# omroot/DeepLearningInAssetPricing_PaperReplication

Measured on AMD Instinct MI355X. Metric: epochs/sec (3-phase GAN), higher is better.
Workload: dtype bf16; 1 GPU; model=Chen-Pelger-Zhu GAN: LSTM[4] + SDF FFN[64,64] + 8 tanh moments, global_batch=1, seq_len=240, panel=T=240/60/300 N=3000 F=46 M=178, bench_config=real, wide_layer0=False, models_per_gpu=1, parallelism=ensemble-dp1, backend=none

## Files before the change

### csrc/k_tbwd.hip

```cpp
#include <algorithm>
#include <type_traits>
#include "common.h"
#include "layout.h"
#include "mlp.h"
#include "tower_dev.h"

typedef short s16x4 __attribute__((ext_vector_type(4)));
typedef uint32_t u32x2 __attribute__((ext_vector_type(2)));
#define LDS3 __attribute__((address_space(3)))

__device__ long long g_tb_ts[8];

namespace {

constexpr int kImg = 4096;
constexpr int kImgs = 3;

DLAP_DEV int img_off(int r, int k) {
  const int f = ((r >> 1) & 1) | (((r >> 3) & 1) << 1), g = (r & 1) << 1;
  return r * 128 + ((((k >> 2) ^ f)) << 5) + (((k & 3) ^ g) << 3);
}

struct ImgMap {
  int wt[4];
  int wx[2];
  int rd[4];
};

DLAP_DEV bf16x8 img_get_sliced(const char* img, int u) {
  const int l = lane_id(), q = l >> 4, n = l & 15;
  const int off = img_off(4 * q + (n >> 2), 4 * u + (n & 3));
  const s16x4 lo = __builtin_amdgcn_ds_read_tr16_b64_v4i16((LDS3 s16x4*)(const_cast<char*>(img) + off));
  const s16x4 hi = __builtin_amdgcn_ds_read_tr16_b64_v4i16((LDS3 s16x4*)(const_cast<char*>(img) + off + 2048));
  typedef short s16x8 __attribute__((ext_vector_type(8)));
  const s16x8 v{lo[0], lo[1], lo[2], lo[3], hi[0], hi[1], hi[2], hi[3]};
  return __builtin_bit_cast(bf16x8, v);
}

DLAP_DEV ImgMap img_map() {
  ImgMap m;
  const int l = lane_id(), q = l >> 4, n = l & 15;
#pragma unroll
  for (int c = 0; c < 4; ++c) m.wt[c] = img_off(n, 4 * c + q);
#pragma unroll
  for (int s = 0; s < 2; ++s) m.wx[s] = img_off(n, 8 * s + 2 * q);
#pragma unroll
  for (int u = 0; u < 4; ++u) m.rd[u] = img_off(8 * q + (n >> 2), 4 * u + (n & 3));
  return m;
}

DLAP_DEV void img_put_t(char* img, const ImgMap& m, const bf16x8 (&f)[2][2]) {
#pragma unroll
  for (int b = 0; b < 2; ++b)
#pragma unroll
    for (int s = 0; s < 2; ++s) {
      const u32x4 v = __builtin_bit_cast(u32x4, f[b][s]);
      *(LDS3 u32x2*)(img + 2048 * b + m.wt[2 * s]) = u32x2{v[0], v[1]};
      *(LDS3 u32x2*)(img + 2048 * b + m.wt[2 * s + 1]) = u32x2{v[2], v[3]};
    }
}
DLAP_DEV void img_put_x(char* img, const ImgMap& m, const bf16x8 (&x)[2][2]) {
#pragma unroll
  for (int b = 0; b < 2; ++b)
#pragma unroll
    for (int s = 0; s < 2; ++s)
      *(LDS3 u32x4*)(img + 2048 * b + m.wx[s]) = __builtin_bit_cast(u32x4, x[b][s]);
}
DLAP_DEV bf16x8 img_get(const char* img, const ImgMap& m, int u) {
  const s16x4 lo = __builtin_amdgcn_ds_read_tr16_b64_v4i16((LDS3 s16x4*)(const_cast<char*>(img) + m.rd[u]));
  const s16x4 hi = __builtin_amdgcn_ds_read_tr16_b64_v4i16((LDS3 s16x4*)(const_cast<char*>(img) + m.rd[u] + 512));
  typedef short s16x8 __attribute__((ext_vector_type(8)));
  const s16x8 v{lo[0], lo[1], lo[2], lo[3], hi[0], hi[1], hi[2], hi[3]};
  return __builtin_bit_cast(bf16x8, v);
}

DLAP_DEV void mma_acc(f32x4& acc, const bf16x8& a, const bf16x8& b) {
  asm("v_mfma_f32_16x16x32_bf16 %0, %1, %2, %0" : "+a"(acc) : "v"(a), "v"(b));
}
DLAP_DEV void acc_fence4(f32x4& a0, f32x4& a1, f32x4& a2, f32x4& a3) {
  asm volatile("s_nop 7\n\ts_nop 7\n\ts_nop 7" : "+a"(a0), "+a"(a1), "+a"(a2), "+a"(a3));
}

__host__ __device__ inline size_t tb_img_base(const MlpDims& D) { return (lds_bytes_of(D) + 15) & ~(size_t)15; }
size_t tb_lds_bytes(const MlpDims& D) {
  const size_t loop = tb_img_base(D) + (size_t)4 * kImgs * kImg;
  const size_t red = (size_t)4 * 4096 * sizeof(float);
  return std::max(loop, red);
}

template <int NL, bool RES>
struct TbW;
template <int NL>
struct TbW<NL, true> {
  bf16x8 w0_[8];
  bf16x8 wf_[NL > 1 ? NL - 1 : 1][8];
  bf16x8 wb_[NL > 1 ? NL - 1 : 1][8];
  bf16x8 wpp_[2];
  DLAP_DEV TbW(const bf16x8* lds, const MlpDims& D) {
#pragma unroll
    for (int k = 0; k < 8; ++k) w0_[k] = ldsf(lds, D.s_fwd0 + k);
#pragma unroll
    for (int j = 0; j + 1 < NL; ++j)
#pragma unroll
      for (int k = 0; k < 8; ++k) {
        wf_[j][k] = ldsf(lds, D.s_fwd + 8 * j + k);
        wb_[j][k] = ldsf(lds, D.s_bwd + 8 * j + k);
      }
#pragma unroll
    for (int k = 0; k < 2; ++k) wpp_[k] = ldsf(lds, D.s_upp + k);
  }
  DLAP_DEV bf16x8 w0(int k) const { return w0_[k]; }
  DLAP_DEV bf16x8 wf(int j, int k) const { return wf_[j][k]; }
  DLAP_DEV bf16x8 wb(int j, int k) const { return wb_[j][k]; }
  DLAP_DEV bf16x8 wpp(int k) const { return wpp_[k]; }
};
template <int NL>
struct TbW<NL, false> {
  const bf16x8* lds;
  const MlpDims& D;
  DLAP_DEV TbW(const bf16x8* l, const MlpDims& d) : lds(l), D(d) {}
  DLAP_DEV bf16x8 w0(int k) const { return ldsf(lds, D.s_fwd0 + k); }
  DLAP_DEV bf16x8 wf(int j, int k) const { return ldsf(lds, D.s_fwd + 8 * j + k); }
  DLAP_DEV bf16x8 wb(int j, int k) const { return ldsf(lds, D.s_bwd + 8 * j + k); }
  DLAP_DEV bf16x8 wpp(int k) const { return ldsf(lds, D.s_upp + k); }
};
template <int NL>
constexpr bool kTbRes = NL <= 2;

template <typename WG>
DLAP_DEV void tb_chain(WG&& wget, const bf16x8 (&pf)[2][2], f32x4 (&acc)[2][4], const float* bias) {
  const int q = lane_id() >> 4;
#pragma unroll
  for (int u = 0; u < 4; ++u) {
    f32x4 c0 = bias ? ld4(bias + 16 * u + 4 * q) : zero4(), c1 = c0;
#pragma unroll
    for (int s = 0; s < 2; ++s) {
      const bf16x8 w = wget(2 * u + s);
      c0 = PrecBF16::mma(w, pf[0][s], c0);
      c1 = PrecBF16::mma(w, pf[1][s], c1);
    }
    acc[0][u] = c0; acc[1][u] = c1;
  }
}

DLAP_DEV void tb_finish(const MlpJob& J, const MlpDims& D, int tile, TileIn<PrecBF16, 2>& in, bf16x8 (&xf)[2][2],
                        const float* spp) {
  const int l = lane_id(), q = l >> 4;
  const int c0 = 32 + 8 * q - D.ppc;
  const bool ins = D.Dm > 0 && c0 >= 0;
  const int ca = max(c0, 0), cb = min(ca + 4, D.ppst - 4);
#pragma unroll
  for (int b = 0; b < 2; ++b) {
    const int r = tile * 32 + 16 * b + (l & 15);
    if (r >= J.R) in.dw[b] = 0.f;
    xf[b][0] = in.x[b][0];
    const float* row = spp + in.ti[b].x * D.ppst;
    const f32x4 v0 = ld4(row + ca), v1 = ld4(row + cb);
    const bf16x8 f = PrecBF16::pack(v0, c0 + 4 < D.ppst ? v1 : zero4());
    xf[b][1] = ins ? f : in.x[b][1];
  }
}

template <int NL>
struct TbState {
  f32x4 dW[NL][4][4];
  f32x4 gb[4];
  f32x4 gwo[4];
  float gbo;
};

template <int NL, bool ZIN, class TI>
DLAP_DEV void tb_tile(const MlpJob& J, const MlpDims& D, const TbW<NL, kTbRes<NL>>& W, const float* aux, const float* spp,
                      char* img, const ImgMap& im, int tile, TI& in, const uint32_t (&kw)[NL],
                      TbState<NL>& S) {
  using P = PrecBF16;
  using Frag = bf16x8;
  const int lane = lane_id(), q = lane >> 4;
  const float* auxt = aux;
  char* ximg = img;
  char* aimg = img + kImg;
  char* zimg = img + 2 * kImg;
  Frag xf[2][2];
  f32x4 a[2][4];
  if constexpr (ZIN) {
    const RowInfo ri = finish_ztile<1>(J, tile, in);
#pragma unroll
    for (int b = 0; b < 2; ++b) {
      xf[b][0] = pp_xfrag<P>(spp, D.ppst, ri.t[b], 0, D);
      xf[b][1] = P::zero();
    }
    img_put_x(ximg, im, xf);
    __builtin_amdgcn_sched_barrier(0);
    zin_sdf0(in.zs, ri, spp, D.ppst, auxt, D, a);
  } else {
    tb_finish(J, D, tile, in, xf, spp);
    img_put_x(ximg, im, xf);
    __builtin_amdgcn_sched_barrier(0);
#pragma unroll
    for (int u = 0; u < 4; ++u) {
      const f32x4 bias = ld4(auxt + D.a_sb + 16 * u + 4 * q);
      f32x4 c0 = bias, c1 = bias;
#pragma unroll
      for (int s = 0; s < 2; ++s) {
        const Frag w = W.w0(2 * u + s);
        c0 = P::mma(w, xf[0][s], c0);
        c1 = P::mma(w, xf[1][s], c1);
      }
      a[0][u] = c0; a[1][u] = c1;
    }
  }
  Frag act[NL][2][2];
  act_tile<P, 4, true>(a, kw[0], act[0]);
#pragma unroll
  for (int j = 1; j < NL; ++j) {
    tb_chain([&](int k) { return W.wf(j - 1, k); }, act[j - 1], a, auxt + D.a_sb + 64 * j);
    act_tile<P, 4, true>(a, kw[j], act[j]);
    __builtin_amdgcn_sched_barrier(0);
  }
  const float dw0 = in.dw[0], dw1 = in.dw[1];
  Frag dzf[2][2];
  {
    f32x4 t[2][4];
#pragma unroll
    for (int u = 0; u < 4; ++u) {
      const f32x4 ww = ld4(auxt + D.a_wo + 16 * u + 4 * q);
      t[0][u] = dw0 * ww;
      t[1][u] = dw1 * ww;
    }
    gate_tile<P, 4>(t, act[NL - 1], dzf);
  }
#pragma unroll
  for (int b = 0; b < 2; ++b)
#pragma unroll
    for (int s = 0; s < 2; ++s) {
      f32x4 lo, hi;
      P::unpack(act[NL - 1][b][s], lo, hi);
      const float d = b ? dw1 : dw0;
      S.gwo[2 * s] += d * lo;
      S.gwo[2 * s + 1] += d * hi;
    }
  S.gbo += q == 0 ? dw0 + dw1 : 0.f;
  __builtin_amdgcn_sched_barrier(0);
#pragma unroll
  for (int j = NL - 1; j >= 0; --j) {
    img_put_t(zimg, im, dzf);
    if (j > 0) img_put_t(aimg, im, act[j - 1]);
    Frag dzN[4];
#pragma unroll
    for (int u = 0; u < 4; ++u) dzN[u] = img_get(zimg, im, u);
    const Frag oh = make_onehot<P>(j);
#pragma unroll
    for (int u = 0; u < 4; ++u) {
      if constexpr (NL == 4) S.gb[u] = P::mma(dzN[u], oh, S.gb[u]);
      else mma_acc(S.gb[u], dzN[u], oh);
    }
#pragma unroll
    for (int v = 0; v < 4; ++v) {
      if (ZIN && j == 0 && v > 0) break;
      const Frag aN = img_get(j > 0 ? aimg : ximg, im, v);
#pragma unroll
      for (int u = 0; u < 4; ++u) mma_acc(S.dW[j][u][v], dzN[u], aN);
    }
    if constexpr (ZIN) {
      if (j == 0) {
        const auto dzo = gp(reinterpret_cast<bf16x8*>(J.dz_out)) + (size_t)tile * 4 * 64 + lane_id();
#pragma unroll
        for (int u = 0; u < 4; ++u) dzo[u * 64] = img_get_sliced(zimg, u);
      }
    }
    __builtin_amdgcn_sched_barrier(0);
    if (j > 0) {
      f32x4 da[2][4];
      tb_chain([&](int k) { return W.wb(j - 1, k); }, dzf, da, nullptr);
      gate_tile<P, 4>(da, act[j - 1], dzf);
    } else if (D.nrnn > 0) {
      f32x4 c[2];
#pragma unroll
      for (int b = 0; b < 2; ++b) {
        c[b] = zero4();
#pragma unroll
        for (int s = 0; s < 2; ++s) c[b] = P::mma(W.wpp(s), dzf[b][s], c[b]);
      }
#pragma unroll
      for (int b = 0; b < 2; ++b) {
        const int row = tile * 32 + 16 * b + (lane & 15);
#pragma unroll
        for (int r = 0; r < 4; ++r) {
          const int d = 4 * q + r;
          if (d < D.Dm && row < J.R) *gp32(J.u_out, (uint32_t)(row * D.Dm + d)) = c[b][r];
        }
      }
    }
  }
}

template <int NL>
DLAP_DEV void tb_issue_kw(const DLAP_GLOBAL uint32_t* gbase, int tile, int ntiles, uint32_t (&kw)[NL]) {
  const int lane = lane_id();
#pragma unroll
  for (int j = 0; j < NL; ++j)
    kw[j] = (gbase && tile < ntiles) ? *at32(gbase, (uint32_t)((tile * NL + j) * 64 + lane)) : 0xFFFFFFFFu;
}

template <int NL>
DLAP_DEV void tb_reduce_store(const MlpJob& J, char* smem, int slab_stride, TbState<NL>& S) {
  const int lane = lane_id(), wave = threadIdx.x >> 6, q = lane >> 4, n = lane & 15;
  float* red = reinterpret_cast<float*>(smem);
  const auto slab = gp(J.slab) + (size_t)(J.slab_base + blockIdx.x) * slab_stride;
#pragma unroll
  for (int j = 0; j < NL; ++j)
#pragma unroll
    for (int u = 0; u < 4; ++u) acc_fence4(S.dW[j][u][0], S.dW[j][u][1], S.dW[j][u][2], S.dW[j][u][3]);
  if constexpr (NL < 4) acc_fence4(S.gb[0], S.gb[1], S.gb[2], S.gb[3]);
  __syncthreads();
#pragma unroll
  for (int j = 0; j < NL; ++j) {
    if (j) __syncthreads();
    float* mine = red + wave * 4096;
#pragma unroll
    for (int u = 0; u < 4; ++u)
#pragma unroll
      for (int v = 0; v < 4; ++v) *reinterpret_cast<f32x4*>(mine + ((4 * u + v) * 64 + lane) * 4) = S.dW[j][u][v];
    __syncthreads();
#pragma unroll
    for (int k = 0; k < 4; ++k) {
      const int pos = (wave * 256 + k * 64 + lane) * 4;
      const f32x4 a = *reinterpret_cast<const f32x4*>(red + pos), b = *reinterpret_cast<const f32x4*>(red + 4096 + pos);
      const f32x4 c = *reinterpret_cast<const f32x4*>(red + 8192 + pos), d = *reinterpret_cast<const f32x4*>(red + 12288 + pos);
      *(DLAP_GLOBAL f32x4*)(slab + j * 4096 + pos) = (a + b) + (c + d);
    }
  }
  __syncthreads();
  float* ex = red + wave * SLAB_EXTRA;
  for (int x = lane; x < SLAB_EXTRA; x += 64) ex[x] = 0.f;
#pragma unroll
  for (int u = 0; u < 4; ++u)
#pragma unroll
    for (int r = 0; r < 4; ++r) {
      const int o = 16 * u + 4 * q + r;
      if (n < NL) ex[64 * n + o] = S.gb[u][r];
      float v = S.gwo[u][r];
      v += __shfl_xor(v, 1, 64); v += __shfl_xor(v, 2, 64);
      v += __shfl_xor(v, 4, 64); v += __shfl_xor(v, 8, 64);
      if (n == 0) ex[64 * DLAP_MAXL + o] = v;
    }
  const float bo = wave_sum(S.gbo);
  if (lane == 0) ex[64 * DLAP_MAXL + 64] = bo;
  __syncthreads();
  for (int x = threadIdx.x; x < SLAB_EXTRA; x += blockDim.x)
    slab[NL * 4096 + x] = (red[x] + red[SLAB_EXTRA + x]) + (red[2 * SLAB_EXTRA + x] + red[3 * SLAB_EXTRA + x]);
}

template <int NL, bool ZIN>
__global__ __launch_bounds__(256, 1) void k_tbwd_sdf(const MlpJob* __restrict__ jobs, MlpDims D, int slab_stride) {
  using P = PrecBF16;
  extern __shared__ __attribute__((aligned(16))) char smem[];
  const MlpJob J = jobs[blockIdx.y];
  bf16x8* lds = reinterpret_cast<bf16x8*>(smem);
  float* aux = aux_lds_ptr(smem, D);
  float* spp = pp_lds_ptr(smem, D);
  const int wave = threadIdx.x >> 6;
  char* img = smem + tb_img_base(D) + (size_t)wave * kImgs * kImg;
  const ImgMap im = img_map();
  const bool tsb = blockIdx.y == 0 && threadIdx.x == 0 && (blockIdx.x == 0 || blockIdx.x == gridDim.x - 1);
  const int tso = blockIdx.x == 0 ? 0 : 4;
  if (tsb) g_tb_ts[tso] = wall_clock64();
  const int ntiles = (J.R + 31) >> 5;
  const int stride = J.nslab * 4;
  const int t0 = blockIdx.x * 4 + wave;
  TbState<NL> S;
#pragma unroll
  for (int j = 0; j < NL; ++j)
#pragma unroll
    for (int u = 0; u < 4; ++u)
#pragma unroll
      for (int v = 0; v < 4; ++v) S.dW[j][u][v] = zero4();
#pragma unroll
  for (int u = 0; u < 4; ++u) { S.gb[u] = zero4(); S.gwo[u] = zero4(); }
  S.gbo = 0.f;
  uint32_t stp_raw = *gp(J.step ? reinterpret_cast<const uint32_t*>(J.step)
                                : reinterpret_cast<const uint32_t*>(J.rowti));
  using TI = std::conditional_t<ZIN, ZTile<1>, TileIn<P, 2>>;
  auto issue = [&](int t, TI& in) {
    if constexpr (ZIN) issue_ztile<1, true>(J, D, t, in, true, false);
    else issue_tile<P, 2, true>(J, t, in);
  };
  TI s0, s1, s2;
  uint32_t k0[NL], k1[NL], k2[NL];
  if (t0 < ntiles) issue(t0, s0);
  if (t0 + stride < ntiles) issue(t0 + stride, s1);
  const bool pre = J.gbits && J.train && J.dropout > 0.f;
  const DLAP_GLOBAL uint32_t* gb0 = pre ? gp(J.gbits) : nullptr;
  const DLAP_GLOBAL uint32_t* gb1 = pre ? gp(J.gbits) + J.gb_half : nullptr;
  uint32_t a0[NL], a1[NL];
  tb_issue_kw<NL>(gb0, t0, ntiles, k0);
  tb_issue_kw<NL>(gb0, t0 + stride, ntiles, k1);
  tb_issue_kw<NL>(gb1, t0, ntiles, a0);
  tb_issue_kw<NL>(gb1, t0 + stride, ntiles, a1);
  stage_weights<P>(J, D, lds, aux, spp);
  asm volatile("" : "+v"(stp_raw));
  const uint32_t stp = J.step ? stp_raw : 0u;
  const DLAP_GLOBAL uint32_t* gbase = (stp & 1u) ? gb1 : gb0;
  if (stp & 1u) {
#pragma unroll
    for (int l = 0; l < NL; ++l) { k0[l] = a0[l]; k1[l] = a1[l]; }
  }
  const TbW<NL, kTbRes<NL>> W(lds, D);
  if (tsb) g_tb_ts[tso + 1] = wall_clock64();
  for (int t = t0; t < ntiles; t += stride) {
    if (t + 2 * stride < ntiles) issue(t + 2 * stride, s2);
    tb_issue_kw<NL>(gbase, t + 2 * stride, ntiles, k2);
    tb_tile<NL, ZIN>(J, D, W, aux, spp, img, im, t, s0, k0, S);
    s0 = s1;
    s1 = s2;
#pragma unroll
    for (int l = 0; l < NL; ++l) { k0[l] = k1[l]; k1[l] = k2[l]; }
  }
  if (tsb) g_tb_ts[tso + 2] = wall_clock64();
  tb_reduce_store<NL>(J, smem, slab_stride, S);
  if (tsb) g_tb_ts[tso + 3] = wall_clock64();
}

}

bool tbwd_supported(const MlpDims& D, int KS1) {
  if (D.wide) return !D.fp32 && D.nl_sdf >= 1 && D.nl_sdf <= 4 && D.Dm >= 1 && D.Dm <= 16;
  return !D.fp32 && KS1 == 2 && D.nl_sdf >= 1 && D.nl_sdf <= 4 && D.Dm <= 16;
}

void launch_tbwd_sdf(const MlpJob* jobs, int njobs, int gx, const MlpDims& D0, int slab_stride, int T,
                     hipStream_t st) {
  MlpDims D = D0;
  D.pp_lds_floats = D.Dm > 0 ? T * D.ppst : 0;
  const size_t sh = tb_lds_bytes(D);
  if (!tbwd_supported(D, 2) || sh > 160 * 1024)
    dlap_throw_hip(hipErrorInvalidValue, "tbwd_sdf: unsupported shape", __FILE__, __LINE__);
  if (slab_stride < D.nl_sdf * 4096 + SLAB_EXTRA)
    dlap_throw_hip(hipErrorInvalidValue, "tbwd_sdf: slab stride too small", __FILE__, __LINE__);
  dim3 grid(gx, njobs), block(256);
#define TB_CASE(N) if (D.nl_sdf == N) { \
    if (D.wide) hipLaunchKernelGGL((k_tbwd_sdf<N, true>), grid, block, sh, st, jobs, D, slab_stride); \
    else hipLaunchKernelGGL((k_tbwd_sdf<N, false>), grid, block, sh, st, jobs, D, slab_stride); \
    HIP_OK(hipGetLastError()); return; }
  TB_CASE(1) TB_CASE(2) TB_CASE(3) TB_CASE(4)
#undef TB_CASE
}

std::vector<long long> tbwd_timestamps() {
  std::vector<long long> v(8);
  HIP_OK(hipMemcpyFromSymbol(v.data(), HIP_SYMBOL(g_tb_ts), sizeof(long long) * 8));
  return v;
}
```

Measured before the change: 7275 model-epochs/s.

## Overlap weight staging and tile prefetch, use packed bf16 relu/gate and DPP reductions

Several changes to the SDF tower backward kernel. A new staging routine loads the weight blob into LDS with direct global-to-LDS loads and overlaps accumulator zeroing with the aux/pp loads. The triple-buffered tile input becomes double-buffered, with the next issue placed right after the current tile's inputs are consumed, which frees registers. It also adds packed-integer bf16 ReLU/dropout and gate ops, vectorized f32x4 stores of u_out when Dm is divisible by 4, and DPP row reductions in place of shuffles. The extra issue placement and register pressure changes may shift scheduling either way.

```diff
diff --git a/csrc/k_tbwd.hip b/csrc/k_tbwd.hip
--- a/csrc/k_tbwd.hip
+++ b/csrc/k_tbwd.hip
@@ -80,6 +80,36 @@
 DLAP_DEV void acc_fence4(f32x4& a0, f32x4& a1, f32x4& a2, f32x4& a3) {
   asm volatile("s_nop 7\n\ts_nop 7\n\ts_nop 7" : "+a"(a0), "+a"(a1), "+a"(a2), "+a"(a3));
 }
+
+struct PrecBF16B : PrecBF16 {
+  template <int SH>
+  DLAP_DEV static uint32_t or_drop_sign(uint32_t nkw, uint32_t v) {
+    uint32_t t;
+    asm("v_pk_lshlrev_b16 %0, %1, %2 op_sel_hi:[0,1]" : "=v"(t) : "i"(15 - SH), "v"(nkw));
+    return (t & 0x80008000u) | v;
+  }
+  template <int BS, bool DROP>
+  DLAP_DEV static Frag act(const f32x4& lo, const f32x4& hi, uint32_t kw) {
+    u32x4 v{cvt_pk(lo[0], lo[1]), cvt_pk(lo[2], lo[3]), cvt_pk(hi[0], hi[1]), cvt_pk(hi[2], hi[3])};
+    if constexpr (DROP) {
+      const uint32_t nkw = ~kw;
+      v[0] = or_drop_sign<BS + 0>(nkw, v[0]); v[1] = or_drop_sign<BS + 1>(nkw, v[1]);
+      v[2] = or_drop_sign<BS + 2>(nkw, v[2]); v[3] = or_drop_sign<BS + 3>(nkw, v[3]);
+    }
+    return __builtin_bit_cast(Frag, u32x4{relu_pk(v[0]), relu_pk(v[1]), relu_pk(v[2]), relu_pk(v[3])});
+  }
+  DLAP_DEV static uint32_t gate_pk(uint32_t d, uint32_t a) {
+    uint32_t nz, r;
+    asm("v_pk_min_u16 %0, %1, 1 op_sel_hi:[1,0]" : "=v"(nz) : "v"(a));
+    asm("v_pk_mul_lo_u16 %0, %1, %2" : "=v"(r) : "v"(d), "v"(nz));
+    return r;
+  }
+  DLAP_DEV static Frag gate(const f32x4& lo, const f32x4& hi, const Frag& a) {
+    const u32x4 av = __builtin_bit_cast(u32x4, a);
+    return __builtin_bit_cast(Frag, u32x4{gate_pk(cvt_pk(lo[0], lo[1]), av[0]), gate_pk(cvt_pk(lo[2], lo[3]), av[1]),
+                                          gate_pk(cvt_pk(hi[0], hi[1]), av[2]), gate_pk(cvt_pk(hi[2], hi[3]), av[3])});
+  }
+};
 
 __host__ __device__ inline size_t tb_img_base(const MlpDims& D) { return (lds_bytes_of(D) + 15) & ~(size_t)15; }
 size_t tb_lds_bytes(const MlpDims& D) {
@@ -169,11 +199,12 @@
   float gbo;
 };
 
-template <int NL, bool ZIN, class TI>
+template <int NL, bool ZIN, class TI, class CONS>
 DLAP_DEV void tb_tile(const MlpJob& J, const MlpDims& D, const TbW<NL, kTbRes<NL>>& W, const float* aux, const float* spp,
                       char* img, const ImgMap& im, int tile, TI& in, const uint32_t (&kw)[NL],
-                      TbState<NL>& S) {
+                      TbState<NL>& S, CONS&& consumed) {
   using P = PrecBF16;
+  using PB = PrecBF16B;
   using Frag = bf16x8;
   const int lane = lane_id(), q = lane >> 4;
   const float* auxt = aux;
@@ -182,6 +213,7 @@
   char* zimg = img + 2 * kImg;
   Frag xf[2][2];
   f32x4 a[2][4];
+  float dw0, dw1;
   if constexpr (ZIN) {
     const RowInfo ri = finish_ztile<1>(J, tile, in);
 #pragma unroll
@@ -192,9 +224,14 @@
     img_put_x(ximg, im, xf);
     __builtin_amdgcn_sched_barrier(0);
     zin_sdf0(in.zs, ri, spp, D.ppst, auxt, D, a);
+    dw0 = in.dw[0]; dw1 = in.dw[1];
+    consumed();
+    __builtin_amdgcn_sched_barrier(0);
   } else {
     tb_finish(J, D, tile, in, xf, spp);
     img_put_x(ximg, im, xf);
+    dw0 = in.dw[0]; dw1 = in.dw[1];
+    consumed();
     __builtin_amdgcn_sched_barrier(0);
 #pragma unroll
     for (int u = 0; u < 4; ++u) {
@@ -210,14 +247,13 @@
     }
   }
   Frag act[NL][2][2];
-  act_tile<P, 4, true>(a, kw[0], act[0]);
+  act_tile<PB, 4, true>(a, kw[0], act[0]);
 #pragma unroll
   for (int j = 1; j < NL; ++j) {
     tb_chain([&](int k) { return W.wf(j - 1, k); }, act[j - 1], a, auxt + D.a_sb + 64 * j);
-    act_tile<P, 4, true>(a, kw[j], act[j]);
+    act_tile<PB, 4, true>(a, kw[j], act[j]);
     __builtin_amdgcn_sched_barrier(0);
   }
-  const float dw0 = in.dw[0], dw1 = in.dw[1];
   Frag dzf[2][2];
   {
     f32x4 t[2][4];
@@ -227,7 +263,7 @@
       t[0][u] = dw0 * ww;
       t[1][u] = dw1 * ww;
     }
-    gate_tile<P, 4>(t, act[NL - 1], dzf);
+    gate_tile<PB, 4>(t, act[NL - 1], dzf);
   }
 #pragma unroll
   for (int b = 0; b < 2; ++b)
@@ -272,7 +308,7 @@
     if (j > 0) {
       f32x4 da[2][4];
       tb_chain([&](int k) { return W.wb(j - 1, k); }, dzf, da, nullptr);
-      gate_tile<P, 4>(da, act[j - 1], dzf);
+      gate_tile<PB, 4>(da, act[j - 1], dzf);
     } else if (D.nrnn > 0) {
       f32x4 c[2];
 #pragma unroll
@@ -281,17 +317,73 @@
 #pragma unroll
         for (int s = 0; s < 2; ++s) c[b] = P::mma(W.wpp(s), dzf[b][s], c[b]);
       }
+      const bool v4 = (D.Dm & 3) == 0;
 #pragma unroll
       for (int b = 0; b < 2; ++b) {
         const int row = tile * 32 + 16 * b + (lane & 15);
-#pragma unroll
-        for (int r = 0; r < 4; ++r) {
-          const int d = 4 * q + r;
-          if (d < D.Dm && row < J.R) *gp32(J.u_out, (uint32_t)(row * D.Dm + d)) = c[b][r];
+        if (v4) {
+          if (4 * q < D.Dm && row < J.R)
+            *(DLAP_GLOBAL f32x4*)gp32(J.u_out, (uint32_t)(row * D.Dm + 4 * q)) = c[b];
+        } else {
+#pragma unroll
+          for (int r = 0; r < 4; ++r) {
+            const int d = 4 * q + r;
+            if (d < D.Dm && row < J.R) *gp32(J.u_out, (uint32_t)(row * D.Dm + d)) = c[b][r];
+          }
         }
       }
     }
   }
+}
+
+template <typename F>
+DLAP_DEV void tb_stage(const MlpJob& J, const MlpDims& D, bf16x8* lds, float* aux, float* spp, F&& in_flight) {
+  const int n16 = D.blob_frags * 64;
+  const auto src = reinterpret_cast<const DLAP_GLOBAL int4*>(gp(J.blob));
+  int4* l16 = reinterpret_cast<int4*>(lds);
+  const int lane = threadIdx.x & 63;
+  for (int i = threadIdx.x; i < n16; i += blockDim.x)
+    __builtin_amdgcn_global_load_lds(src + i, (LDS3 void*)(l16 + (i - lane)), 16, 0, 0);
+  constexpr int B = 8;
+  const int nthr = blockDim.x;
+  const auto ga = gp(J.aux);
+  const auto gpp = gp(J.pp);
+  const int n = (D.pp_lds_floats > 0 && D.Dm > 0) ? J.T * D.ppst : 0;
+  const int pst = max(D.ppst, 1);
+  const int dt = nthr / pst, dc = nthr - dt * pst;
+  int t = (int)threadIdx.x / pst, c = (int)threadIdx.x - t * pst;
+  float va[B], vp[B];
+#pragma unroll
+  for (int k = 0; k < B; ++k) {
+    const int i = threadIdx.x + k * nthr;
+    va[k] = ga[i < D.aux_floats ? i : 0];
+  }
+#pragma unroll
+  for (int k = 0; k < B; ++k) {
+    const int i = threadIdx.x + k * nthr;
+    vp[k] = (i < n && c < D.Dm) ? gpp[t * D.Dm + c] : 0.f;
+    t += dt; c += dc;
+    if (c >= pst) { c -= pst; ++t; }
+  }
+  in_flight();
+#pragma unroll
+  for (int k = 0; k < B; ++k) {
+    const int i = threadIdx.x + k * nthr;
+    if (i < D.aux_floats) aux[i] = va[k];
+  }
+#pragma unroll
+  for (int k = 0; k < B; ++k) {
+    const int i = threadIdx.x + k * nthr;
+    if (i < n) spp[i] = vp[k];
+  }
+  for (int i = threadIdx.x + B * nthr; i < D.aux_floats; i += nthr) aux[i] = ga[i];
+  for (int i = threadIdx.x + B * nthr; i < n; i += nthr) {
+    spp[i] = c < D.Dm ? gpp[t * D.Dm + c] : 0.f;
+    t += dt; c += dc;
+    if (c >= pst) { c -= pst; ++t; }
+  }
+  asm volatile("s_waitcnt vmcnt(0)" ::: "memory");
+  __syncthreads();
 }
 
 template <int NL>
@@ -300,6 +392,18 @@
 #pragma unroll
   for (int j = 0; j < NL; ++j)
     kw[j] = (gbase && tile < ntiles) ? *at32(gbase, (uint32_t)((tile * NL + j) * 64 + lane)) : 0xFFFFFFFFu;
+}
+
+template <int CTRL>
+DLAP_DEV float dpp_row(float x) {
+  return __int_as_float(__builtin_amdgcn_update_dpp(0, __float_as_int(x), CTRL, 0xF, 0xF, false));
+}
+DLAP_DEV float row16_sum(float v) {
+  v += dpp_row<0xB1>(v);
+  v += dpp_row<0x4E>(v);
+  v += dpp_row<0x141>(v);
+  v += dpp_row<0x140>(v);
+  return v;
 }
 
 template <int NL>
@@ -339,9 +443,7 @@
     for (int r = 0; r < 4; ++r) {
       const int o = 16 * u + 4 * q + r;
       if (n < NL) ex[64 * n + o] = S.gb[u][r];
-      float v = S.gwo[u][r];
-      v += __shfl_xor(v, 1, 64); v += __shfl_xor(v, 2, 64);
-      v += __shfl_xor(v, 4, 64); v += __shfl_xor(v, 8, 64);
+      const float v = row16_sum(S.gwo[u][r]);
       if (n == 0) ex[64 * DLAP_MAXL + o] = v;
     }
   const float bo = wave_sum(S.gbo);
@@ -369,15 +471,6 @@
   const int stride = J.nslab * 4;
   const int t0 = blockIdx.x * 4 + wave;
   TbState<NL> S;
-#pragma unroll
-  for (int j = 0; j < NL; ++j)
-#pragma unroll
-    for (int u = 0; u < 4; ++u)
-#pragma unroll
-      for (int v = 0; v < 4; ++v) S.dW[j][u][v] = zero4();
-#pragma unroll
-  for (int u = 0; u < 4; ++u) { S.gb[u] = zero4(); S.gwo[u] = zero4(); }
-  S.gbo = 0.f;
   uint32_t stp_raw = *gp(J.step ? reinterpret_cast<const uint32_t*>(J.step)
                                 : reinterpret_cast<const uint32_t*>(J.rowti));
   using TI = std::conditional_t<ZIN, ZTile<1>, TileIn<P, 2>>;
@@ -385,7 +478,7 @@
     if constexpr (ZIN) issue_ztile<1, true>(J, D, t, in, true, false);
     else issue_tile<P, 2, true>(J, t, in);
   };
-  TI s0, s1, s2;
+  TI s0, s1;
   uint32_t k0[NL], k1[NL], k2[NL];
   if (t0 < ntiles) issue(t0, s0);
   if (t0 + stride < ntiles) issue(t0 + stride, s1);
@@ -397,7 +490,29 @@
   tb_issue_kw<NL>(gb0, t0 + stride, ntiles, k1);
   tb_issue_kw<NL>(gb1, t0, ntiles, a0);
   tb_issue_kw<NL>(gb1, t0 + stride, ntiles, a1);
-  stage_weights<P>(J, D, lds, aux, spp);
+  auto zero_sums = [&]() __attribute__((always_inline)) {
+#pragma unroll
+    for (int j = 0; j < NL; ++j)
+#pragma unroll
+      for (int u = 0; u < 4; ++u)
+#pragma unroll
+        for (int v = 0; v < 4; ++v) {
+          S.dW[j][u][v] = zero4();
+          if constexpr (NL < 4) asm volatile("" : "+a"(S.dW[j][u][v]));
+        }
+#pragma unroll
+    for (int u = 0; u < 4; ++u) {
+      S.gb[u] = zero4(); S.gwo[u] = zero4();
+      if constexpr (NL < 4) asm volatile("" : "+a"(S.gb[u]));
+    }
+    S.gbo = 0.f;
+  };
+  if constexpr (NL < 4) {
+    tb_stage(J, D, lds, aux, spp, zero_sums);
+  } else {
+    zero_sums();
+    stage_weights<P>(J, D, lds, aux, spp);
+  }
   asm volatile("" : "+v"(stp_raw));
   const uint32_t stp = J.step ? stp_raw : 0u;
   const DLAP_GLOBAL uint32_t* gbase = (stp & 1u) ? gb1 : gb0;
@@ -408,11 +523,11 @@
   const TbW<NL, kTbRes<NL>> W(lds, D);
   if (tsb) g_tb_ts[tso + 1] = wall_clock64();
   for (int t = t0; t < ntiles; t += stride) {
-    if (t + 2 * stride < ntiles) issue(t + 2 * stride, s2);
     tb_issue_kw<NL>(gbase, t + 2 * stride, ntiles, k2);
-    tb_tile<NL, ZIN>(J, D, W, aux, spp, img, im, t, s0, k0, S);
-    s0 = s1;
-    s1 = s2;
+    tb_tile<NL, ZIN>(J, D, W, aux, spp, img, im, t, s0, k0, S, [&] {
+      s0 = s1;
+      if (t + 2 * stride < ntiles) issue(t + 2 * stride, s1);
+    });
 #pragma unroll
     for (int l = 0; l < NL; ++l) { k0[l] = k1[l]; k1[l] = k2[l]; }
   }
```

New measurement: 7441 model-epochs/s (median of 6 runs). 2.3% higher.
